# lashhw/rtcuda

Measured on AMD Instinct MI355X. Metric: Msamples/s at 1920x1080, bun_zipper.ply, higher is better.
Workload: dtype f32

## Files before the change

### rtcuda_amd/api.py

```python
from __future__ import annotations

import ctypes
import dataclasses
import os
import subprocess

import numpy as np

from .scenes import SceneArrays

_PKG = os.path.dirname(os.path.abspath(__file__))
LIB_PATH = os.path.join(_PKG, os.environ.get("RT_LIB_NAME", "librtcuda_amd.so"))
CSRC = os.path.join(_PKG, "csrc")

W = 1 << 20
FLAG_TIME_KERNELS = 1
FLAG_DETERMINISTIC = 2
FLAG_RNG_PER_SAMPLE = 4
FLAG_REFERENCE_WALK = 8
SCENE_DEVICE_BVH = 1
FLAG_WATERTIGHT = 16
AOV_CHANNELS = 11
AOV_ALBEDO, AOV_NORMAL, AOV_EMISSION, AOV_DEPTH, AOV_HITS = 0, 3, 6, 9, 10

# ... 20 lines not shown


class RtStats(ctypes.Structure):
    _fields_ = [
        ("camera_rays", ctypes.c_int64), ("shade_events", ctypes.c_int64), ("closest_rays", ctypes.c_int64),
        ("any_rays", ctypes.c_int64), ("emission_adds", ctypes.c_int64), ("shadow_adds", ctypes.c_int64),
        ("rr_draws", ctypes.c_int64), ("iterations", ctypes.c_int64), ("bvh_nodes", ctypes.c_int64),
        ("bvh_depth", ctypes.c_int64), ("seconds_render", ctypes.c_double), ("seconds_rng_init", ctypes.c_double),
        ("seconds_trace", ctypes.c_double), ("seconds_reference_tree", ctypes.c_double), ("seconds_advance", ctypes.c_double),
        ("launches_trace", ctypes.c_int64), ("reserved", ctypes.c_int64 * 7),
    ]

    def as_dict(self) -> dict:
        d = {n: getattr(self, n) for n, _ in self._fields_ if n != "reserved"}
        d["lds_top_records"] = int(self.reserved[2])
        d["slot_chunk"] = max(int(self.reserved[1]) - 1, 0)
        d["literal_retraces"], d["reference_lost_hits"], d["exact_ties"] = (int(self.reserved[k]) for k in (4, 5, 6))
        return d


class RtDenoiseParams(ctypes.Structure):
    _fields_ = [("passes", ctypes.c_int32), ("sigma_color", ctypes.c_float), ("sigma_depth", ctypes.c_float),
                ("normal_power_log2", ctypes.c_int32), ("flags", ctypes.c_uint32)]


class RtDenoiseDualParams(ctypes.Structure):
    _fields_ = [("passes", ctypes.c_int32), ("sigma_variance", ctypes.c_float), ("sigma_depth", ctypes.c_float),
                ("normal_power_log2", ctypes.c_int32), ("flags", ctypes.c_uint32)]


def build(verbose: bool = False) -> str:
# ... 813 lines not shown
```

### rtcuda_amd/csrc/rt_frame_kernels.inc

```

template <bool LDS_TABLES>
__global__ void __launch_bounds__(kBlock)
RT_K_ADVANCE(DScene sc, DPools p, RT_FRAME_SRC cam, AdvanceParams ap, float *__restrict__ fb, DCounters *__restrict__ ctr,
             DWaveRow *__restrict__ rows, unsigned int *__restrict__ lock_shades) {
    if (ap.lockstep >= 3 && lock_shades[ap.lockstep - 2] == 0u) return;
    __shared__ float s_tab[LDS_TABLES ? kTabDwordsMax : 1];
    const int i = blockIdx.x * blockDim.x + threadIdx.x;
    const bool in_range = i < ap.n;
    SlotState st;
    st.bounces = kDone;
    st.hit_info = -1;
    st.pixel = 0;
    st.gen = 0;
    st.rs = Rng{0, 0, 0, 0, 0, 0};
    st.beta = st.wo = st.isect_p = st.isect_n = mk(0, 0, 0);
    if (in_range) {
        st.bounces = p.bounces(i);
        st.hit_info = p.hit_info(i);
        st.pixel = p.pixel(i);
        st.gen = p.gen(i);
        st.rs = Rng{p.rd(i), p.r0(i), p.r1(i), p.r2(i), p.r3(i), p.r4(i)};
        st.beta = mk(p.br(i), p.bg(i), p.bb(i));
        st.wo = mk(p.dx(i), p.dy(i), p.dz(i));
        st.isect_p = mk(p.hpx(i), p.hpy(i), p.hpz(i));
// ... 84 lines not shown
           int prio_period, int rot_wave, int rot_set, int gen_batch, int tri_follow, unsigned int *__restrict__ next_cid,
           unsigned long long *__restrict__ vstat) {
    constexpr bool SPLIT_GEN = MIN_WAVES != 2;
    asm volatile("s_nop 0\n\ts_nop 0");
    extern __shared__ int s_lds[];
    int *stack = s_lds + threadIdx.x;
    float *park = (float *)(s_lds + (stack_cap + 1) * kBlock) + threadIdx.x;
    int *over = overflow + (blockIdx.x * kBlock + threadIdx.x) % kOverStride;
    int *cold = s_lds + (stack_cap + 10) * kBlock + threadIdx.x;
    float *acc = (float *)(s_lds + (stack_cap + 23) * kBlock) + threadIdx.x;
    float *s_tab = (float *)(s_lds + (stack_cap + 26) * kBlock);
    const float *tab = sc.tables;
    const float4 *s_top = (const float4 *)(s_tab + (LDS_TABLES ? ((sc.tab_dwords + 3) & ~3) : 0));
    constexpr bool CHUNKS = RT_PATHS_CHUNKS && SPLIT_GEN && !DRAW_CIDS;
    __shared__ __attribute__((aligned(16))) unsigned s_task[CHUNKS ? 8 : 1];
    if (CHUNKS && threadIdx.x == 0) {
        const rtchunks::Multiple m = rtchunks::multiple_of(top_n > 0 ? (unsigned)top_n : 1u);
        s_task[0] = 0u;
        s_task[1] = top_n > 0 ? (unsigned)top_n : 0u;
        s_task[2] = m.inv;
        s_task[3] = m.shift;
        s_task[4] = m.limit;
    }
    const bool chunk_start = CHUNKS && top_n > 0;
    if (MIN_WAVES != 2) top_n = 0;
    for (int k = threadIdx.x; k < top_n * 4; k += kBlock) ((float4 *)s_top)[k] = sc.nodes[k];
    if (LDS_TABLES) {
        for (int k = threadIdx.x; k < sc.tab_dwords; k += kBlock) s_tab[k] = sc.tables[k];
        tab = s_tab;
    }
    struct Uniforms {
        RT_FRAME_SRC cam;
        AdvanceParams ap;
    };
    static_assert(sizeof(Uniforms) % 4 == 0, "dword copy");
    Uniforms *s_uni = (Uniforms *)(s_top + 4 * (size_t)top_n);
    {
        Uniforms u;
        u.cam = cam_arg;
// ... 88 lines not shown
    acc[0 * kBlock] = acc[1 * kBlock] = acc[2 * kBlock] = 0.f;
    if (chunk_start) {
        i = ap_n;
        phase = PH_GEN;
        cold[12 * kBlock] = -1;
    } else if (i < ap_n) {
        load_slot(i);
        phase = (bounces != kDone && bounces != kParked) ? (SPLIT_GEN ? PH_GEN : PH_ADV) : PH_IDLE;
        cold_save();
        cold[12 * kBlock] = -1;
    }
    unsigned long long n_gen = 0, n_shade = 0, n_traced = 0, n_shadow = 0, n_emit = 0, n_deposit = 0, n_rr = 0;
#ifdef RT_TRACE_PROFILE
    unsigned long long pf[16] = {0, 0, 0, 0, 0, 0, 0, 0, 0, 0, 0, 0, 0, 0, 0, 0};
    unsigned long long pf_gen_cycles = 0, pf_fin_cycles = 0, pf_fin_lanes = 0, pf_fin_iters = 0;
    const unsigned long long pf_t0 = __builtin_readcyclecounter();
    unsigned long long pf_last_work = 0;
#endif

    unsigned prio_tick = 0;
    const unsigned prio_rank = (4u * blockIdx.x) / gridDim.x;
    while (true) {
        RT_MARK("loop.head");
        if (prio_period && (prio_tick++ & ((1u << prio_period) - 1u)) == 0u) {
            unsigned lvl = ((prio_tick >> prio_period) + prio_rank) & 3u;
            lvl = max(lvl, prio_rank >> 1);
            switch (lvl) {
                case 0: __builtin_amdgcn_s_setprio(0); break;
                case 1: __builtin_amdgcn_s_setprio(1); break;
                case 2: __builtin_amdgcn_s_setprio(2); break;
// ... 36 lines not shown
                while (served < need) {
                    if (cid_next == cid_end) {
                        unsigned base = 0;
                        if (lane_id() == 0) base = atomicAdd(next_cid, (unsigned)kCidChunk);
                        static_assert(0x7ffff000u + (unsigned)kCidChunk < 0x7fffffffu, "cid_end must not overflow int");
                        cid_next = (int)min(__builtin_amdgcn_readfirstlane(base), 0x7ffff000u);
                        cid_end = cid_next + kCidChunk;
                    }
                    const int take = min(need - served, cid_end - cid_next);
                    if (phase == PH_GEN && rank >= served && rank < served + take) my_cid = cid_next + (rank - served);
                    cid_next += take;
                    served += take;
                }
            }
            const unsigned chunk_g = CHUNKS ? __builtin_amdgcn_readfirstlane(s_task[1]) : 0u;
            if (CHUNKS && chunk_g) {
                const rtchunks::Multiple chunk_m{s_task[2], s_task[3], s_task[4]};
                bool need = phase == PH_GEN && i >= ap_n;
                const bool at_end = phase == PH_GEN && i < ap_n &&
                                    rtchunks::chunk_ends((unsigned)cold[2 * kBlock], chunk_m, cold[0 * kBlock] == kChunkFresh);
                if (wave_ballot(need || at_end)) {
                    if (at_end) {
                        cold_load();
                        const bool ends = gen == ap.last_gen || (long long)gen * kW + (ap.slot_lo + i) >= ap.cam_end;
                        if (!ends) {
                            acc_flush(acc, fb, ap_fb_fixed, pixel);
                            bounces = ap_max_bounces;
                            store_slot(i);
                            const int old = __hip_atomic_fetch_add(&p.sem(i), 1, __ATOMIC_RELEASE, __HIP_MEMORY_SCOPE_WORKGROUP);
                            if (!rtchunks::runner_keeps(old)) {
                                i = ap_n;
                                need = true;
                            }
                        }
                    }
                    const unsigned chunk_sets = (unsigned)ap_n / (unsigned)lanes_in_grid;
                    const unsigned chunk_tasks = rtchunks::task_count(chunk_sets, (unsigned)ap.last_gen, (unsigned)chunk_g);
                    unsigned long long m;
                    while ((m = wave_ballot(need)) != 0ull) {
                        unsigned base = 0;
                        if (lane_id() == 0) base = atomicAdd(&s_task[0], (unsigned)__popcll(m));
                        const unsigned t = __builtin_amdgcn_readfirstlane(base) + prefix_popc(m);
                        if (need) {
                            if (t >= chunk_tasks) {
                                need = false;
                                phase = PH_IDLE;
                            } else {
                                const rtchunks::Entry e = rtchunks::task_entry(t, chunk_sets);
                                const int k = slot_of((int)e.set, e.lane);
                                const int old = k < ap_n ? __hip_atomic_fetch_sub(&p.sem(k), 1, __ATOMIC_ACQUIRE, __HIP_MEMORY_SCOPE_WORKGROUP) : 0;
                                if (rtchunks::taker_runs(old)) {
                                    i = k;
                                    load_slot(i);
                                    cold_save();
                                    cold[0 * kBlock] = kChunkFresh;
                                    cold[12 * kBlock] = -1;
                                    need = false;
                                }
                            }
                        }
                    }
                }
            }
            if (phase == PH_GEN) {
                SlotState st;
                st.gen = cold[2 * kBlock];
                st.rs = Rng{(uint32_t)cold[3 * kBlock], (uint32_t)cold[4 * kBlock], (uint32_t)cold[5 * kBlock],
                            (uint32_t)cold[6 * kBlock], (uint32_t)cold[7 * kBlock], (uint32_t)cold[8 * kBlock]};
                st.bounces = 0;
                st.pixel = 0;
                st.beta = mk(0, 0, 0);
                int pxy = cold[12 * kBlock];
                acc_flush(acc, fb, ap_fb_fixed, cold[1 * kBlock]);
                gen_core<true>(cam, ap, ap.slot_lo + i, st, out, &pxy, my_cid);
                cold[0 * kBlock] = st.bounces;
                cold[2 * kBlock] = st.gen;
                cold[3 * kBlock] = (int)st.rs.d;
                cold[4 * kBlock] = (int)st.rs.v0;
                cold[5 * kBlock] = (int)st.rs.v1;
                cold[6 * kBlock] = (int)st.rs.v2;
                cold[7 * kBlock] = (int)st.rs.v3;
                cold[8 * kBlock] = (int)st.rs.v4;
                if (out.new_ray) {
                    cold[1 * kBlock] = st.pixel;
                    cold[9 * kBlock] = __float_as_int(st.beta.x);
                    cold[10 * kBlock] = __float_as_int(st.beta.y);
                    cold[11 * kBlock] = __float_as_int(st.beta.z);
                    cold[12 * kBlock] = pxy;
// ... 2 lines not shown
                }
            }
            const bool nr = out.new_ray;
            o = out.ray_o;
            d = out.ray_d;
            inv = inv_dir(d);
            phase = nr ? (int)PH_CLOSEST : phase;
            tmax = nr ? kFltMax : tmax;
            tri = nr ? -1 : tri;
            cur = nr ? 0 : cur;
            sp = nr ? 0 : sp;
            if (wave_ballot(hand_back)) {
                if (hand_back) {
                    if (draw_cids) {
                        phase = PH_IDLE;
                    } else if (CHUNKS && chunk_g) {
                        cold_load();
                        store_slot(i);
                        i = ap_n;
                        tri = -1;
                    } else {
                        next_slot(PH_GEN);
                    }
                }
            }
            n_gen += wave_count((out.did_gen));
            n_traced += wave_count((out.new_ray));
#ifdef RT_TRACE_PROFILE
            pf_gen_cycles += __builtin_readcyclecounter() - pf_tg;
#endif
            retake();
            RT_MARK("gen.end");
        }
        if (run_adv) {
#ifdef RT_TRACE_PROFILE
// ... 275 lines not shown
        pf_last_work = phase != PH_IDLE ? pf_tf - pf_t0 : pf_last_work;
#endif
    }
#ifdef RT_TRACE_PROFILE
    if (prof && lane_id() == 0) { atomicAdd(&prof[17], pf_fin_cycles); atomicAdd(&prof[18], pf_fin_lanes); atomicAdd(&prof[19], pf_fin_iters); }
    const unsigned long long pf_life = __builtin_readcyclecounter() - pf_t0;
    unsigned long long pf_idle = pf_life - pf_last_work, pf_idle_max = pf_idle;
    for (int off = 32; off > 0; off >>= 1) {
        pf_idle += __shfl_xor(pf_idle, off);
        const unsigned long long other = __shfl_xor(pf_idle_max, off);
        pf_idle_max = other > pf_idle_max ? other : pf_idle_max;
    }
    if (prof && lane_id() == 0)
        { pf[11] = pf_life; for (int k = 0; k < 16; k++) atomicAdd(&prof[k], pf[k]); atomicMax(&prof[13], pf[11]); atomicAdd(&prof[14], 1ull); atomicAdd(&prof[16], pf_gen_cycles);
          atomicAdd(&prof[20], pf_idle); atomicAdd(&prof[21], pf_idle_max);
          unsigned long long *rec = prof + 24 + kProfRec * (size_t)((blockIdx.x * kBlock + threadIdx.x) >> 6);
          rec[0] = __builtin_amdgcn_s_getreg((31 << 11) | 4);
          rec[1] = __builtin_amdgcn_s_getreg((31 << 11) | 20);
          rec[2] = pf[11];
          rec[3] = pf[0] + pf[2] + pf[4];
          rec[4] = pf_idle;
          rec[5] = pf_idle_max; }
#endif
    unsigned long long v[C_COUNT] = {n_gen, n_shade, n_traced, n_shadow, n_emit, n_deposit, n_rr, 0ull};
    row_add(rows, v);
}
```

### rtcuda_amd/csrc/rt_host_check.cpp

```cpp
#include <cfloat>
#include <cmath>
#include <cstdint>
#include <cstdio>
#include <cstring>
#include <cstdlib>
#include <vector>

#include "rt_bvh.h"
#include "rt_denoise.h"
#include "rt_launch_plan.h"
#include "rt_ploc.h"
#include "rt_ref_tree.h"
#include "rt_slot_chunks.h"
#include "rt_stats_merge.h"

namespace {
struct V3 { float x, y, z; };
inline V3 sub(V3 a, V3 b) { return {a.x - b.x, a.y - b.y, a.z - b.z}; }
inline float dot(V3 a, V3 b) { return a.x * b.x + a.y * b.y + a.z * b.z; }
inline V3 cross(V3 a, V3 b) { return {a.y * b.z - a.z * b.y, a.z * b.x - a.x * b.z, a.x * b.y - a.y * b.x}; }
struct Tri { V3 p0, e1, e2, n; };
inline bool tri_hit(const Tri &tr, V3 o, V3 d, float tmax, float &t) {
    V3 c = sub(tr.p0, o);
    V3 r = cross(d, c);
// ... 837 lines not shown
        slots[k] = rtchunks::slot_of(e.set, (unsigned)block * rtchunks::kLanes + e.lane, (unsigned)lanes_in_grid, (unsigned)rot_wave, (unsigned)rot_set);
        levels[k] = (int32_t)e.level;
    }
}
int rt_slot_chunk_static_slot(int set, int lane_in_grid, int lanes_in_grid, int rot_wave, int rot_set) {
    return rtchunks::slot_of((unsigned)set, (unsigned)lane_in_grid, (unsigned)lanes_in_grid, (unsigned)rot_wave, (unsigned)rot_set);
}
uint32_t rt_slot_chunk_levels(uint32_t rays, uint32_t G) { return rtchunks::levels(rays, G); }
uint32_t rt_slot_chunk_task_count(uint32_t sets, uint32_t rays, uint32_t G) { return rtchunks::task_count(sets, rays, G); }
int rt_slot_chunk_ends(uint32_t gen, uint32_t G, int fresh) { return rtchunks::chunk_ends(gen, rtchunks::multiple_of(G), fresh != 0); }
int rt_slot_chunk_taker_runs(int old_sem) { return rtchunks::taker_runs(old_sem); }
int rt_slot_chunk_runner_keeps(int old_sem) { return rtchunks::runner_keeps(old_sem); }
int rt_plan_slot_chunk(int n, int cus, int chain) {
    return rtplan::slot_chunk_for(rtplan::plan_paths_launch(n, cus, true, 70000, 10, true, 1920, 256, 0), chain);
}
int hc_denoise(const int64_t *sum_fixed, int num_samples, const int64_t *aov_fixed, int aov_samples, int width, int height, int passes,
               float sigma_color, float sigma_depth, int normal_power_log2, float *rgb_out) {
    if (!sum_fixed || !aov_fixed || !rgb_out || width < 1 || height < 1 || num_samples < 1 || aov_samples < 1) return 1;
    if (passes < 0 || passes > DN_MAX_PASSES || normal_power_log2 < 0 || normal_power_log2 > DN_MAX_NORMAL_POWER_LOG2) return 1;
    if (!(std::isfinite(sigma_color) && sigma_color > 0.f && std::isfinite(sigma_depth) && sigma_depth > 0.f)) return 1;
    const float sc2 = sigma_color * sigma_color, sd2 = sigma_depth * sigma_depth;
    const float kz = 1.f / sd2;
    float kc[DN_MAX_PASSES];
    for (int i = 0; i < passes; i++) {
        kc[i] = (float)(1 << (2 * i)) / sc2;
        if (!(std::isfinite(kc[i]) && kc[i] > 0.f)) return 1;
    }
    if (!(std::isfinite(kz) && kz > 0.f)) return 1;
    const size_t n = (size_t)width * (size_t)height;
    const float inv_spp = 1.f / (float)num_samples, inv_aov = 1.f / (float)aov_samples;
// ... 44 lines not shown
```

### rtcuda_amd/csrc/rt_host_render.inc

```
struct Context {
    int device = -1;
    int n = 0;
    int lane = 0;
    DPools pools{};
    std::vector<void *> allocs;
    DCounters *d_ctr = nullptr;
    DCounters *h_ctr = nullptr;
    DWaveRow *d_rows = nullptr;
    int n_rows = 0;
    uint32_t *d_jump = nullptr;
    hipEvent_t ev_ring[4] = {nullptr, nullptr, nullptr, nullptr};
    hipEvent_t ev_a = nullptr, ev_b = nullptr, ev_c = nullptr;
    uint64_t rng_seed = 0;
    int rng_lo = -1;
    bool rng_valid = false;
    uint32_t *rng_backup = nullptr;
    std::vector<hipEvent_t> timing_events;
    unsigned int *d_lock = nullptr;
    int lock_cap = 0;
    int *d_over = nullptr;
    int over_levels = 0;
    std::mutex busy;
    Context() = default;
    Context(const Context &) = delete;
// ... 206 lines not shown
    RayTable table;
    long long n_rays;
    bool keyed = false;
    KeyedRayTable keyed_table{};
};
struct FrameRun {
    Context &c;
    const rt_scene *scene;
    const RayFrame *rays;
    hipStream_t st;
    float *d_sum;
    uint32_t flags;
    bool per_sample;
    HitMode mode;
    bool lds_tables = false, persistent = true, finished = false, ran_lockstep = false;
    int cus = 0, stack_cap = 0, top_records_in_lds = 0, slot_chunk = 0, lock_enqueued = 0;
    DScene sc{};
    Camera cam{};
    AdvanceParams ap{};
    TraceParams tpp{};
    size_t lds_bytes = 0, ev_used = 0;
    dim3 grid_trace;
    TraceKernel trace = nullptr;
    hipEvent_t ev_start = nullptr, ev_stop = nullptr;
    long long rounds = 0;
    float ms_paths = 0.f;
    double rng_seconds = 0.0, ref_tree_seconds = 0.0;
    ~FrameRun() {
        if (ev_start) (void)hipEventDestroy(ev_start);
        if (ev_stop) (void)hipEventDestroy(ev_stop);
    }
// ... 12 lines not shown
        }
        *out = c.timing_events[ev_used++];
        return 0;
    }
};

#ifdef RT_TRACE_PROFILE
static int report_paths_profile(unsigned long long *paths_prof, int paths_blocks) {
    unsigned long long h[24];
    HIP_TRY(hipMemcpy(h, paths_prof, 192, hipMemcpyDeviceToHost));
    fprintf(stderr, "k_paths cycles: ADV %.1f%% (%.0f / block) node %.1f%% (%.0f) tri %.1f%% (%.0f) rest %.1f%%\n",
            100.0 * h[8] / h[11], h[0] ? (double)h[8] / h[0] : 0.0, 100.0 * h[9] / h[11], h[2] ? (double)h[9] / h[2] : 0.0,
            100.0 * h[10] / h[11], h[4] ? (double)h[10] / h[4] : 0.0, 100.0 * (double)(h[11] - h[8] - h[9] - h[10]) / h[11]);
    fprintf(stderr, "k_paths GEN blocks: %llu avg lanes %.1f, %.1f %% of wave time (%.0f cycles / block; inside `rest` above)\n", h[12],
            h[12] ? (double)h[15] / h[12] : 0.0, 100.0 * h[16] / h[11], h[12] ? (double)h[16] / h[12] : 0.0);
    fprintf(stderr, "k_paths waves: %llu, mean lifetime %.0f cycles, longest %.0f cycles (x%.3f)\n", h[14], (double)h[11] / h[14], (double)h[13],
            (double)h[13] * h[14] / h[11]);
    fprintf(stderr, "k_paths lane-idle tail: %.2f %% of wave time x 64 lanes; a wave's first lane is idle for good %.2f %% of the wave's time before its exit\n",
            100.0 * h[20] / (64.0 * h[11]), 100.0 * h[21] / h[11]);
    fprintf(stderr, "k_paths fin section: %.1f %% of wave time, entered in %llu iterations (avg %.1f finished lanes), %.0f cycles each\n",
            100.0 * h[17] / h[11], h[19], h[19] ? (double)h[18] / h[19] : 0.0, h[19] ? (double)h[17] / h[19] : 0.0);
    fprintf(stderr, "k_paths profile: ADV blocks %llu avg lanes %.1f | node steps %llu avg lanes %.1f (ADV-waiting %.1f) | tri steps %llu avg lanes %.1f (ADV-waiting %.1f)\n",
            h[0], h[0] ? (double)h[1] / h[0] : 0.0, h[2], h[2] ? (double)h[3] / h[2] : 0.0, h[2] ? (double)h[6] / h[2] : 0.0, h[4],
            h[4] ? (double)h[5] / h[4] : 0.0, h[4] ? (double)h[7] / h[4] : 0.0);
    if (const char *dump = knob("RT_PROF_DUMP")) {
        std::vector<unsigned long long> recs(kProfRec * (size_t)paths_blocks * (kBlock / 64));
        HIP_TRY(hipMemcpy(recs.data(), paths_prof + 24, recs.size() * 8, hipMemcpyDeviceToHost));
        if (FILE *f = fopen(dump, "w")) {
            for (size_t k = 0; k < recs.size(); k += kProfRec)
                fprintf(f, "%zu %llu %llu %llu %llu %llu %llu\n", k / kProfRec, recs[k], recs[k + 1], recs[k + 2], recs[k + 3], recs[k + 4], recs[k + 5]);
// ... 20 lines not shown
    const size_t fixed_lds = (lds_tables ? sizeof(float) * (size_t)((scene->tab_dwords + 3) & ~3) : 0) + sizeof(Camera) + sizeof(AdvanceParams);
    const rtplan::PathsLaunch p = rtplan::plan_paths_launch(c.n, cus, scene->wide, scene->n_nodes, paths_cap, !rays, ap.width, ap.spp, fixed_lds);
    top_records_in_lds = p.top_n;
    unsigned long long *paths_prof = nullptr;
#ifdef RT_TRACE_PROFILE
    const size_t prof_bytes = 192 + 8 * kProfRec * (size_t)(grid_for(c.n) * (kBlock / 64));
    HIP_TRY(hipMalloc((void **)&paths_prof, prof_bytes));
    HIP_TRY(hipMemset(paths_prof, 0, prof_bytes));
#endif
    auto launch_paths = [&](auto kernel, const auto &src, int top_n) {
        hipLaunchKernelGGL(kernel, dim3(p.blocks), dim3(kBlock), p.lds_bytes, st, sc, c.pools, src, ap, d_sum, c.d_rows, paths_cap, c.d_over,
                           p.adv_batch, (flags & 0x100u) ? 1 : 0, paths_prof, top_n, p.prio_rotate, p.rot_wave, p.rot_set, p.gen_batch, p.tri_follow, &c.d_ctr->pad2[0],
                           &c.d_ctr->vstat[0]);
    };
    HIP_TRY(hipEventRecord(c.ev_a, st));
    const int chunk = (rays || p.few_blocks || per_sample || ap.last_gen < 1 || ap.n != c.n) ? 0 : rtplan::slot_chunk_for(p, ap.last_gen);
    slot_chunk = chunk;
    if (rays && rays->keyed) launch_paths(paths_keyed_kernel(lds_tables, p.few_blocks), rays->keyed_table, p.top_n);
    else if (rays) launch_paths(paths_rays_kernel(lds_tables, p.few_blocks, mode.verify), rays->table, p.top_n);
    else if (chunk > 0) launch_paths(paths_chunked_kernel(lds_tables, scene->wide, mode.literal, mode.verify), cam, chunk);
    else launch_paths(paths_kernel(lds_tables, scene->wide, p.few_blocks, per_sample, mode.literal, mode.verify), cam, mode.literal ? 0 : p.top_n);
    HIP_TRY(hipGetLastError());
    HIP_TRY(hipEventRecord(c.ev_b, st));
    HIP_TRY(hipEventSynchronize(c.ev_b));
    HIP_TRY(hipEventElapsedTime(&ms_paths, c.ev_a, c.ev_b));
#ifdef RT_TRACE_PROFILE
    if (report_paths_profile(paths_prof, p.blocks)) return 1;
#endif
    finished = true;
    return 0;
}

int FrameRun::run_rounds() {
    const int kBatch = 8;
    const int kTimeStride = 4;
// ... 112 lines not shown
    stats->bvh_nodes = scene->n_nodes;
    stats->bvh_depth = scene->max_depth;
    stats->seconds_render = ms_total * 1e-3;
    stats->seconds_rng_init = rng_seconds;
    double scale_up = n_sampled > 0 ? (double)rounds / (double)n_sampled : 0.0;
    stats->seconds_trace = t_ch * 1e-3 * scale_up;
    stats->seconds_reference_tree = ref_tree_seconds;
    stats->seconds_advance = t_adv * 1e-3 * scale_up;
    stats->launches_trace = rounds;
    stats->reserved[0] = n_sampled;
    if (persistent) {
        stats->seconds_trace = ms_paths * 1e-3;
        stats->seconds_advance = 0.0;
        stats->launches_trace = 1;
        stats->reserved[0] = 1;
        stats->reserved[1] = 1 + slot_chunk;
        stats->reserved[2] = top_records_in_lds;
    }
    rare_path_counters(h_final.vstat, &stats->reserved[4]);
    return 0;
}

int render_shard_impl(const rt_scene *scene, const rt_camera *camera, int width, int height, int spp,
                      int max_bounces, uint64_t seed, int shard_index, int shard_count, uint32_t flags,
                      float *d_sum, hipStream_t st, rt_stats *stats, int ctx_lane = 0, const RayFrame *rays = nullptr) {
    if (!scene || (!camera && !rays) || !d_sum) return fail("rt_render_shard: null argument");
    if (width <= 0 || height <= 0 || spp <= 0 || max_bounces < 0) return fail("rt_render_shard: bad dimensions");
    if (max_bounces > (1 << 24)) return fail("rt_render_shard: max_bounces exceeds 16777216");
    if (shard_count <= 0 || kW % shard_count != 0 || shard_index < 0 || shard_index >= shard_count)
        return fail("rt_render_shard: shard_count must divide 1048576 and 0 <= shard_index < shard_count");
    if ((long long)width * height > (long long)(0x7fffffff / 3))
// ... 389 lines not shown
```

### rtcuda_amd/csrc/rt_launch_plan.h

```cpp
#pragma once

#include <algorithm>
#include <cstdlib>

#include "rt_bvh.h"

namespace rtplan {
constexpr int kBlock = 256, kSlots = 1 << 20;

struct PathsLaunch {
    int blocks;
    bool few_blocks;
    size_t lds_bytes;
    int top_n, adv_batch, gen_batch, tri_follow, prio_rotate, rot_wave, rot_set;
    int slot_chunk;
};
constexpr int kSlotChunkAuto = -1, kChunksPerSlot = 8, kChunkChainLo = 384, kChunkChainHi = 768;

inline PathsLaunch plan_paths_launch(int n, int cus, bool wide, int n_nodes, int paths_cap, bool lattice, int width, int spp,
                                     size_t fixed_lds_bytes) {
    using rtbvh::knob;
    PathsLaunch p{};
    p.lds_bytes = sizeof(int) * (size_t)kBlock * (size_t)(paths_cap + 26) + fixed_lds_bytes;
    p.blocks = (n + kBlock - 1) / kBlock;
    {
        int want = 1024;
        if (const char *e = knob("RT_PATHS_BLOCKS")) want = std::max(1, atoi(e));
        while (p.blocks > want && p.blocks % 2 == 0) p.blocks /= 2;
    }
    p.few_blocks = p.blocks <= 2 * cus;
    if (p.few_blocks) {
        const int prefix = std::min(n_nodes, (int)rtbvh::kTopPrefix * (wide ? 2 : 1));
// ... 19 lines not shown
            while (b) { long long t = a % b; a = b; b = t; }
            period = a * (spp / 64);
        }
        const int waves = p.blocks * (kBlock / 64);
        if (period < 16 || period > waves) period = std::max(16, waves / 8);
        p.rot_wave = (int)(period / 4);
        p.rot_set = (int)(period / 4 + period / 16);
        if (const char *e = knob("RT_ROT_WAVE")) p.rot_wave = atoi(e);
        if (const char *e = knob("RT_ROT_SET")) p.rot_set = atoi(e);
        p.rot_wave &= ~3;
    }
    if (const char *e = knob("RT_PRIO_ROTATE")) p.prio_rotate = atoi(e);
    p.slot_chunk = (p.few_blocks || n / (p.blocks * kBlock) < 2) ? 0 : kSlotChunkAuto;
    if (const char *e = knob("RT_SLOT_CHUNK")) p.slot_chunk = p.few_blocks ? 0 : std::max(0, std::min(1 << 20, atoi(e)));
    if (n % (p.blocks * kBlock) != 0) p.slot_chunk = 0;
    return p;
}
inline int slot_chunk_for(const PathsLaunch &p, int chain) {
    if (p.slot_chunk != kSlotChunkAuto) return p.slot_chunk;
    if (chain < kChunkChainLo || chain > kChunkChainHi) return 0;
    return (chain + kChunksPerSlot - 1) / kChunksPerSlot;
}
}
```

### rtcuda_amd/csrc/rt_slot_chunks.h

```cpp
#pragma once

#if defined(__HIPCC__)
#define RT_CHUNKS_FN __host__ __device__ inline
#else
#define RT_CHUNKS_FN inline
#endif

namespace rtchunks {
constexpr unsigned kLanes = 256;

RT_CHUNKS_FN unsigned levels(unsigned rays, unsigned G) { return (rays + G - 1u) / G; }
RT_CHUNKS_FN unsigned task_count(unsigned sets, unsigned rays, unsigned G) { return sets * kLanes * levels(rays, G); }

struct Entry {
    unsigned set, lane, level;
};
RT_CHUNKS_FN Entry task_entry(unsigned t, unsigned sets) {
    const unsigned S = sets * kLanes, idx = t % S;
    return Entry{idx / kLanes, idx % kLanes, t / S};
}

RT_CHUNKS_FN int slot_of(unsigned set, unsigned lane_in_grid, unsigned lanes_in_grid, unsigned rot_wave, unsigned rot_set) {
    const unsigned wave_in_grid = lane_in_grid >> 6, lane_in_wave = lane_in_grid & 63u;
    const unsigned b = (wave_in_grid + (wave_in_grid & 3u) * rot_wave + set * rot_set) & ((lanes_in_grid >> 6) - 1u);
    return (int)(set * lanes_in_grid + b * 64u + lane_in_wave);
}

RT_CHUNKS_FN bool taker_runs(int old_sem) { return old_sem >= 1; }
RT_CHUNKS_FN bool runner_keeps(int old_sem) { return old_sem < 0; }

struct Multiple {
    unsigned inv, shift, limit;
};
RT_CHUNKS_FN Multiple multiple_of(unsigned G) {
    unsigned shift = 0;
    while (((G >> shift) & 1u) == 0u) shift++;
    const unsigned odd = G >> shift;
    unsigned inv = odd;
    for (int k = 0; k < 5; k++) inv *= 2u - odd * inv;
    return Multiple{inv, shift, 0xffffffffu / G};
}
RT_CHUNKS_FN bool is_multiple(unsigned gen, const Multiple &m) {
    const unsigned q = gen * m.inv;
    return ((q >> m.shift) | (m.shift ? q << (32u - m.shift) : 0u)) <= m.limit;
}
// ... 3 lines not shown
```

### rtcuda_amd/csrc/rtcuda_amd.hip

```cpp
#include <hip/hip_runtime.h>

#include <algorithm>
#include <chrono>
#include <cmath>
#include <cstdio>
#include <cstring>
#include <memory>
#include <mutex>
#include <thread>
#include <type_traits>
#include <string>
#include <vector>

#include "../../include/rtcuda_amd.h"
#include "rt_bvh.h"
#include "rt_denoise.h"
#include "rt_device.h"
#include "rt_launch_plan.h"
#include "rt_ploc.h"
#include "rt_ref_tree.h"
#include "rt_slot_chunks.h"
#include "rt_stats_merge.h"

using namespace rt;
// ... 39 lines not shown
    const float *tables;
    int tab_dwords;
    const float4 *ref_nodes;
    const int *ref_prims;
    int ref_n_prims;
    const int *ref_leaf_of;
    const int *ref_parent;
    int ref_root_leaf;
};
__device__ __host__ inline int tab_off_lights(int n_mats) { return 5 * n_mats; }
__device__ __host__ inline int tab_off_ltri(int n_mats, int n_lights) { return 5 * n_mats + 8 * n_lights; }
__device__ __host__ inline int tab_off_lpre(int n_mats, int n_lights) { return 5 * n_mats + 20 * n_lights; }
constexpr int kTabPerMat = 5, kTabPerLight = 8 + 12 + 4;
inline int tab_dwords(int n_mats, int n_lights) { return kTabPerMat * n_mats + kTabPerLight * n_lights; }

enum { A_OX, A_OY, A_OZ, A_DX, A_DY, A_DZ, A_HPX, A_HPY, A_HPZ, A_HNX, A_HNY, A_HNZ, A_BR, A_BG, A_BB, A_SOX, A_SOY, A_SOZ, A_SDX, A_SDY, A_SDZ, A_STMAX, A_SLR, A_SLG, A_SLB, A_HIT_INFO, A_BOUNCES, A_PIXEL, A_GEN, A_STARGET, A_RD, A_R0, A_R1, A_R2, A_R3, A_R4, A_SEM, A_COUNT };
struct DPools {
    float *base;
    int n;
    __device__ __forceinline__ float &ox(int i) const { return base[(unsigned)(A_OX * n + i)]; }
    __device__ __forceinline__ float &oy(int i) const { return base[(unsigned)(A_OY * n + i)]; }
    __device__ __forceinline__ float &oz(int i) const { return base[(unsigned)(A_OZ * n + i)]; }
    __device__ __forceinline__ float &dx(int i) const { return base[(unsigned)(A_DX * n + i)]; }
    __device__ __forceinline__ float &dy(int i) const { return base[(unsigned)(A_DY * n + i)]; }
    __device__ __forceinline__ float &dz(int i) const { return base[(unsigned)(A_DZ * n + i)]; }
    __device__ __forceinline__ float &hpx(int i) const { return base[(unsigned)(A_HPX * n + i)]; }
    __device__ __forceinline__ float &hpy(int i) const { return base[(unsigned)(A_HPY * n + i)]; }
    __device__ __forceinline__ float &hpz(int i) const { return base[(unsigned)(A_HPZ * n + i)]; }
    __device__ __forceinline__ float &hnx(int i) const { return base[(unsigned)(A_HNX * n + i)]; }
    __device__ __forceinline__ float &hny(int i) const { return base[(unsigned)(A_HNY * n + i)]; }
    __device__ __forceinline__ float &hnz(int i) const { return base[(unsigned)(A_HNZ * n + i)]; }
// ... 9 lines not shown
    __device__ __forceinline__ float &stmax(int i) const { return base[(unsigned)(A_STMAX * n + i)]; }
    __device__ __forceinline__ float &slr(int i) const { return base[(unsigned)(A_SLR * n + i)]; }
    __device__ __forceinline__ float &slg(int i) const { return base[(unsigned)(A_SLG * n + i)]; }
    __device__ __forceinline__ float &slb(int i) const { return base[(unsigned)(A_SLB * n + i)]; }
    __device__ __forceinline__ int &hit_info(int i) const { return ((int *)base)[(unsigned)(A_HIT_INFO * n + i)]; }
    __device__ __forceinline__ int &bounces(int i) const { return ((int *)base)[(unsigned)(A_BOUNCES * n + i)]; }
    __device__ __forceinline__ int &pixel(int i) const { return ((int *)base)[(unsigned)(A_PIXEL * n + i)]; }
    __device__ __forceinline__ int &gen(int i) const { return ((int *)base)[(unsigned)(A_GEN * n + i)]; }
    __device__ __forceinline__ int &starget(int i) const { return ((int *)base)[(unsigned)(A_STARGET * n + i)]; }
    __device__ __forceinline__ uint32_t &rd(int i) const { return ((uint32_t *)base)[(unsigned)(A_RD * n + i)]; }
    __device__ __forceinline__ uint32_t &r0(int i) const { return ((uint32_t *)base)[(unsigned)(A_R0 * n + i)]; }
    __device__ __forceinline__ uint32_t &r1(int i) const { return ((uint32_t *)base)[(unsigned)(A_R1 * n + i)]; }
    __device__ __forceinline__ uint32_t &r2(int i) const { return ((uint32_t *)base)[(unsigned)(A_R2 * n + i)]; }
    __device__ __forceinline__ uint32_t &r3(int i) const { return ((uint32_t *)base)[(unsigned)(A_R3 * n + i)]; }
    __device__ __forceinline__ uint32_t &r4(int i) const { return ((uint32_t *)base)[(unsigned)(A_R4 * n + i)]; }
    __device__ __forceinline__ int &sem(int i) const { return ((int *)base)[(unsigned)(A_SEM * n + i)]; }
    float *array(int k) const { return base + (size_t)k * n; }
};

struct DCounters {
    int last_live_round;
    unsigned int unused0;
    unsigned int pad2[2];
    unsigned long long vstat[4];
};
enum { V_OWN_FAIL = 0, V_LOST = 1, V_TIE = 2, V_LITERAL = 3 };
enum { C_CAMERA = 0, C_SHADE, C_CLOSEST, C_ANY, C_EMIT, C_SHADOW_ADD, C_RR, C_UNUSED, C_COUNT };
struct DWaveRow {
    unsigned long long c[C_COUNT];
};

// ... 46 lines not shown
    p.rd(i) = seed_state.d;
    p.r0(i) = v[0];
    p.r1(i) = v[1];
    p.r2(i) = v[2];
    p.r3(i) = v[3];
    p.r4(i) = v[4];
}

__global__ void k_pool_init(DPools p, int n, int max_bounces) {
    int i = blockIdx.x * blockDim.x + threadIdx.x;
    if (i >= n) return;
    p.hit_info(i) = -1;
    p.bounces(i) = max_bounces;
    p.gen(i) = 0;
    p.pixel(i) = 0;
    p.sem(i) = 1;
}

struct AdvanceParams {
    int n;
    int slot_lo;
    int width, height, spp, max_bounces;
    long long cam_end;
    int round;
    int batch_mask;
    int last_gen;
    int lockstep;
    int fb_fixed;
    int w_over_spp;
    int dpx, dpy;
    int per_sample, key_mul, key_add;
// ... 770 lines not shown
```

Baseline: 5053.

## Move chunk hand-off semaphores into LDS and deal only the tail slot sets

Replaces the per-slot global semaphore array with packed 16-bit LDS semaphore fields, so release and acquire become workgroup-local LDS atomics instead of global memory atomics. Chunked dealing now applies only to the last few slot sets (a 'head' offset packed into top_n), and the accumulator flush is deferred until after the hand-off. Chunking is disabled unless occupancy allows enough resident workgroups per CU. The catch is that hand-offs are restricted to within a workgroup and to fewer sets, and there is an extra waitcnt before the release atomic.

Result: faster. 5110, median of 6 (+1.1%).

```diff
diff --git a/rtcuda_amd/api.py b/rtcuda_amd/api.py
--- a/rtcuda_amd/api.py
+++ b/rtcuda_amd/api.py
@@ -58,7 +58,8 @@
     def as_dict(self) -> dict:
         d = {n: getattr(self, n) for n, _ in self._fields_ if n != "reserved"}
         d["lds_top_records"] = int(self.reserved[2])
-        d["slot_chunk"] = max(int(self.reserved[1]) - 1, 0)
+        d["slot_chunk"] = max((int(self.reserved[1]) & 0xffffffff) - 1, 0)
+        d["slot_head"] = int(self.reserved[1]) >> 32
         d["literal_retraces"], d["reference_lost_hits"], d["exact_ties"] = (int(self.reserved[k]) for k in (4, 5, 6))
         return d
 
diff --git a/rtcuda_amd/csrc/rt_frame_kernels.inc b/rtcuda_amd/csrc/rt_frame_kernels.inc
--- a/rtcuda_amd/csrc/rt_frame_kernels.inc
+++ b/rtcuda_amd/csrc/rt_frame_kernels.inc
@@ -1,3 +1,6 @@
+#ifndef RT_CHUNK_RELEASE_WAIT
+#define RT_CHUNK_RELEASE_WAIT 1
+#endif
 
 template <bool LDS_TABLES>
 __global__ void __launch_bounds__(kBlock)
@@ -122,15 +125,22 @@
     const float4 *s_top = (const float4 *)(s_tab + (LDS_TABLES ? ((sc.tab_dwords + 3) & ~3) : 0));
     constexpr bool CHUNKS = RT_PATHS_CHUNKS && SPLIT_GEN && !DRAW_CIDS;
     __shared__ __attribute__((aligned(16))) unsigned s_task[CHUNKS ? 8 : 1];
-    if (CHUNKS && threadIdx.x == 0) {
-        const rtchunks::Multiple m = rtchunks::multiple_of(top_n > 0 ? (unsigned)top_n : 1u);
-        s_task[0] = 0u;
-        s_task[1] = top_n > 0 ? (unsigned)top_n : 0u;
-        s_task[2] = m.inv;
-        s_task[3] = m.shift;
-        s_task[4] = m.limit;
-    }
-    const bool chunk_start = CHUNKS && top_n > 0;
+    __shared__ unsigned s_sem[CHUNKS ? rtchunks::kSemWords : 1];
+    const unsigned chunk_g0 = (CHUNKS && top_n > 0) ? (unsigned)top_n & ((1u << rtplan::kChunkHeadShift) - 1u) : 0u;
+    const unsigned chunk_head0 = (CHUNKS && top_n > 0) ? (unsigned)top_n >> rtplan::kChunkHeadShift : 0u;
+    if (CHUNKS) {
+        for (unsigned k = threadIdx.x; k < rtchunks::kSemWords; k += kBlock) s_sem[k] = rtchunks::kSemWordInit;
+        if (threadIdx.x == 0) {
+            const rtchunks::Multiple m = rtchunks::multiple_of(chunk_g0 ? chunk_g0 : 1u);
+            s_task[0] = 0u;
+            s_task[1] = chunk_g0;
+            s_task[2] = m.inv;
+            s_task[3] = m.shift;
+            s_task[4] = m.limit;
+            s_task[5] = chunk_head0;
+        }
+    }
+    const bool chunk_start = CHUNKS && chunk_g0 && chunk_head0 == 0u;
     if (MIN_WAVES != 2) top_n = 0;
     for (int k = threadIdx.x; k < top_n * 4; k += kBlock) ((float4 *)s_top)[k] = sc.nodes[k];
     if (LDS_TABLES) {
@@ -249,6 +259,7 @@
 #ifdef RT_TRACE_PROFILE
     unsigned long long pf[16] = {0, 0, 0, 0, 0, 0, 0, 0, 0, 0, 0, 0, 0, 0, 0, 0};
     unsigned long long pf_gen_cycles = 0, pf_fin_cycles = 0, pf_fin_lanes = 0, pf_fin_iters = 0;
+    unsigned long long pf_handovers = 0, pf_handover_blocks = 0;
     const unsigned long long pf_t0 = __builtin_readcyclecounter();
     unsigned long long pf_last_work = 0;
 #endif
@@ -315,27 +326,45 @@
                 }
             }
             const unsigned chunk_g = CHUNKS ? __builtin_amdgcn_readfirstlane(s_task[1]) : 0u;
+            const bool chunk_was_gen = CHUNKS && phase == PH_GEN;
+            const int chunk_acc_pixel = CHUNKS ? cold[1 * kBlock] : 0;
             if (CHUNKS && chunk_g) {
                 const rtchunks::Multiple chunk_m{s_task[2], s_task[3], s_task[4]};
+                const unsigned chunk_head = __builtin_amdgcn_readfirstlane(s_task[5]);
                 bool need = phase == PH_GEN && i >= ap_n;
-                const bool at_end = phase == PH_GEN && i < ap_n &&
+                const bool at_end = phase == PH_GEN && i < ap_n && slot_set >= (int)chunk_head &&
                                     rtchunks::chunk_ends((unsigned)cold[2 * kBlock], chunk_m, cold[0 * kBlock] == kChunkFresh);
                 if (wave_ballot(need || at_end)) {
+#ifdef RT_TRACE_PROFILE
+                    bool pf_released = false;
+#endif
                     if (at_end) {
                         cold_load();
                         const bool ends = gen == ap.last_gen || (long long)gen * kW + (ap.slot_lo + i) >= ap.cam_end;
                         if (!ends) {
-                            acc_flush(acc, fb, ap_fb_fixed, pixel);
                             bounces = ap_max_bounces;
                             store_slot(i);
-                            const int old = __hip_atomic_fetch_add(&p.sem(i), 1, __ATOMIC_RELEASE, __HIP_MEMORY_SCOPE_WORKGROUP);
-                            if (!rtchunks::runner_keeps(old)) {
+                            const rtchunks::Owner own = rtchunks::owner_of((unsigned)i, (unsigned)lanes_in_grid, (unsigned)rot_wave, (unsigned)rot_set);
+                            const unsigned idx = (own.set - chunk_head) * rtchunks::kLanes + (own.lane_in_grid & (rtchunks::kLanes - 1u));
+#if RT_CHUNK_RELEASE_WAIT
+                            __builtin_amdgcn_s_waitcnt(0x0f70);
+#endif
+                            const unsigned old = __hip_atomic_fetch_add(&s_sem[rtchunks::sem_word(idx) & (rtchunks::kSemWords - 1u)], rtchunks::sem_unit(idx),
+                                                                        __ATOMIC_RELEASE, __HIP_MEMORY_SCOPE_WORKGROUP);
+                            if (!rtchunks::runner_keeps(rtchunks::sem_value(old, idx))) {
                                 i = ap_n;
                                 need = true;
                             }
+#ifdef RT_TRACE_PROFILE
+                            pf_released = true;
+#endif
                         }
                     }
-                    const unsigned chunk_sets = (unsigned)ap_n / (unsigned)lanes_in_grid;
+#ifdef RT_TRACE_PROFILE
+                    pf_handovers += wave_count(pf_released);
+                    pf_handover_blocks += wave_ballot(pf_released) != 0 ? 1 : 0;
+#endif
+                    const unsigned chunk_sets = (unsigned)ap_n / (unsigned)lanes_in_grid - chunk_head;
                     const unsigned chunk_tasks = rtchunks::task_count(chunk_sets, (unsigned)ap.last_gen, (unsigned)chunk_g);
                     unsigned long long m;
                     while ((m = wave_ballot(need)) != 0ull) {
@@ -348,9 +377,12 @@
                                 phase = PH_IDLE;
                             } else {
                                 const rtchunks::Entry e = rtchunks::task_entry(t, chunk_sets);
-                                const int k = slot_of((int)e.set, e.lane);
-                                const int old = k < ap_n ? __hip_atomic_fetch_sub(&p.sem(k), 1, __ATOMIC_ACQUIRE, __HIP_MEMORY_SCOPE_WORKGROUP) : 0;
-                                if (rtchunks::taker_runs(old)) {
+                                const int k = slot_of((int)(e.set + chunk_head), e.lane);
+                                const unsigned idx = e.set * rtchunks::kLanes + e.lane;
+                                const unsigned old = k < ap_n ? __hip_atomic_fetch_sub(&s_sem[rtchunks::sem_word(idx) & (rtchunks::kSemWords - 1u)], rtchunks::sem_unit(idx),
+                                                                                       __ATOMIC_ACQUIRE, __HIP_MEMORY_SCOPE_WORKGROUP)
+                                                              : rtchunks::kSemBias;
+                                if (rtchunks::taker_runs(rtchunks::sem_value(old, idx))) {
                                     i = k;
                                     load_slot(i);
                                     cold_save();
@@ -363,6 +395,10 @@
                     }
                 }
             }
+            if (CHUNKS) {
+                __builtin_amdgcn_s_waitcnt(0x0f70);
+                if (chunk_was_gen) acc_flush(acc, fb, ap_fb_fixed, chunk_acc_pixel);
+            }
             if (phase == PH_GEN) {
                 SlotState st;
                 st.gen = cold[2 * kBlock];
@@ -372,7 +408,7 @@
                 st.pixel = 0;
                 st.beta = mk(0, 0, 0);
                 int pxy = cold[12 * kBlock];
-                acc_flush(acc, fb, ap_fb_fixed, cold[1 * kBlock]);
+                if (!CHUNKS) acc_flush(acc, fb, ap_fb_fixed, cold[1 * kBlock]);
                 gen_core<true>(cam, ap, ap.slot_lo + i, st, out, &pxy, my_cid);
                 cold[0 * kBlock] = st.bounces;
                 cold[2 * kBlock] = st.gen;
@@ -405,11 +441,12 @@
                 if (hand_back) {
                     if (draw_cids) {
                         phase = PH_IDLE;
-                    } else if (CHUNKS && chunk_g) {
+                    } else if (CHUNKS && chunk_g && slot_set + 1 >= (int)s_task[5]) {
                         cold_load();
                         store_slot(i);
                         i = ap_n;
                         tri = -1;
+                        slot_set = (int)s_task[5];
                     } else {
                         next_slot(PH_GEN);
                     }
@@ -715,6 +752,7 @@
     if (prof && lane_id() == 0)
         { pf[11] = pf_life; for (int k = 0; k < 16; k++) atomicAdd(&prof[k], pf[k]); atomicMax(&prof[13], pf[11]); atomicAdd(&prof[14], 1ull); atomicAdd(&prof[16], pf_gen_cycles);
           atomicAdd(&prof[20], pf_idle); atomicAdd(&prof[21], pf_idle_max);
+          atomicAdd(&prof[22], pf_handovers); atomicAdd(&prof[23], pf_handover_blocks);
           unsigned long long *rec = prof + 24 + kProfRec * (size_t)((blockIdx.x * kBlock + threadIdx.x) >> 6);
           rec[0] = __builtin_amdgcn_s_getreg((31 << 11) | 4);
           rec[1] = __builtin_amdgcn_s_getreg((31 << 11) | 20);
diff --git a/rtcuda_amd/csrc/rt_host_check.cpp b/rtcuda_amd/csrc/rt_host_check.cpp
--- a/rtcuda_amd/csrc/rt_host_check.cpp
+++ b/rtcuda_amd/csrc/rt_host_check.cpp
@@ -875,6 +875,30 @@
 int rt_plan_slot_chunk(int n, int cus, int chain) {
     return rtplan::slot_chunk_for(rtplan::plan_paths_launch(n, cus, true, 70000, 10, true, 1920, 256, 0), chain);
 }
+int rt_plan_slot_head(int n, int cus, int *sets_out) {
+    const rtplan::PathsLaunch p = rtplan::plan_paths_launch(n, cus, true, 70000, 10, true, 1920, 256, 0);
+    const int sets = n / (p.blocks * rtplan::kBlock);
+    if (sets_out) *sets_out = sets;
+    return rtplan::slot_head_for(p, sets);
+}
+int rt_plan_slot_chunk_if_resident(int chunk, int workgroups_per_cu) { return rtplan::slot_chunk_if_resident(chunk, workgroups_per_cu); }
+void rt_slot_chunk_head_tasks(int block, int sets, int head, int lanes_in_grid, int rot_wave, int rot_set, uint32_t t0, int count, int32_t *slots, int32_t *levels, int32_t *idx) {
+    for (int k = 0; k < count; k++) {
+        const rtchunks::Entry e = rtchunks::task_entry(t0 + (uint32_t)k, (unsigned)(sets - head));
+        slots[k] = rtchunks::slot_of(e.set + (unsigned)head, (unsigned)block * rtchunks::kLanes + e.lane, (unsigned)lanes_in_grid, (unsigned)rot_wave, (unsigned)rot_set);
+        levels[k] = (int32_t)e.level;
+        idx[k] = (int32_t)(e.set * rtchunks::kLanes + e.lane);
+    }
+}
+void rt_slot_chunk_owner(int slot, int lanes_in_grid, int rot_wave, int rot_set, int32_t *out2) {
+    const rtchunks::Owner o = rtchunks::owner_of((unsigned)slot, (unsigned)lanes_in_grid, (unsigned)rot_wave, (unsigned)rot_set);
+    out2[0] = (int32_t)o.set;
+    out2[1] = (int32_t)o.lane_in_grid;
+}
+uint32_t rt_slot_chunk_sem_word(uint32_t idx) { return rtchunks::sem_word(idx); }
+uint32_t rt_slot_chunk_sem_unit(uint32_t idx) { return rtchunks::sem_unit(idx); }
+int rt_slot_chunk_sem_value(uint32_t word, uint32_t idx) { return rtchunks::sem_value(word, idx); }
+uint32_t rt_slot_chunk_sem_init() { return rtchunks::kSemWordInit; }
 int hc_denoise(const int64_t *sum_fixed, int num_samples, const int64_t *aov_fixed, int aov_samples, int width, int height, int passes,
                float sigma_color, float sigma_depth, int normal_power_log2, float *rgb_out) {
     if (!sum_fixed || !aov_fixed || !rgb_out || width < 1 || height < 1 || num_samples < 1 || aov_samples < 1) return 1;
diff --git a/rtcuda_amd/csrc/rt_host_render.inc b/rtcuda_amd/csrc/rt_host_render.inc
--- a/rtcuda_amd/csrc/rt_host_render.inc
+++ b/rtcuda_amd/csrc/rt_host_render.inc
@@ -244,7 +244,7 @@
     bool per_sample;
     HitMode mode;
     bool lds_tables = false, persistent = true, finished = false, ran_lockstep = false;
-    int cus = 0, stack_cap = 0, top_records_in_lds = 0, slot_chunk = 0, lock_enqueued = 0;
+    int cus = 0, stack_cap = 0, top_records_in_lds = 0, slot_chunk = 0, slot_head = 0, lock_enqueued = 0;
     DScene sc{};
     Camera cam{};
     AdvanceParams ap{};
@@ -287,6 +287,8 @@
             100.0 * h[10] / h[11], h[4] ? (double)h[10] / h[4] : 0.0, 100.0 * (double)(h[11] - h[8] - h[9] - h[10]) / h[11]);
     fprintf(stderr, "k_paths GEN blocks: %llu avg lanes %.1f, %.1f %% of wave time (%.0f cycles / block; inside `rest` above)\n", h[12],
             h[12] ? (double)h[15] / h[12] : 0.0, 100.0 * h[16] / h[11], h[12] ? (double)h[16] / h[12] : 0.0);
+    fprintf(stderr, "k_paths GEN cycles per wave %.0f; chunked deal: %.2f hand-overs per lane, made in %.2f %% of the GEN blocks\n", h[14] ? (double)h[16] / h[14] : 0.0,
+            h[14] ? (double)h[22] / (64.0 * h[14]) : 0.0, h[12] ? 100.0 * h[23] / h[12] : 0.0);
     fprintf(stderr, "k_paths waves: %llu, mean lifetime %.0f cycles, longest %.0f cycles (x%.3f)\n", h[14], (double)h[11] / h[14], (double)h[13],
             (double)h[13] * h[14] / h[11]);
     fprintf(stderr, "k_paths lane-idle tail: %.2f %% of wave time x 64 lanes; a wave's first lane is idle for good %.2f %% of the wave's time before its exit\n",
@@ -337,11 +339,19 @@
                            &c.d_ctr->vstat[0]);
     };
     HIP_TRY(hipEventRecord(c.ev_a, st));
-    const int chunk = (rays || p.few_blocks || per_sample || ap.last_gen < 1 || ap.n != c.n) ? 0 : rtplan::slot_chunk_for(p, ap.last_gen);
+    int chunk = (rays || p.few_blocks || per_sample || ap.last_gen < 1 || ap.n != c.n) ? 0 : rtplan::slot_chunk_for(p, ap.last_gen);
+    const PathsKernel chunked = paths_chunked_kernel(lds_tables, scene->wide, mode.literal, mode.verify);
+    if (chunk > 0) {
+        int per_cu = 0;
+        HIP_TRY(hipOccupancyMaxActiveBlocksPerMultiprocessor(&per_cu, chunked, kBlock, p.lds_bytes));
+        chunk = rtplan::slot_chunk_if_resident(chunk, per_cu);
+    }
+    slot_head = chunk > 0 ? rtplan::slot_head_for(p, ap.n / (p.blocks * kBlock)) : 0;
+    static_assert(rtplan::kDealtSetsMax == (int)rtchunks::kDealtSetsMax, "the plan deals what the semaphores hold");
     slot_chunk = chunk;
     if (rays && rays->keyed) launch_paths(paths_keyed_kernel(lds_tables, p.few_blocks), rays->keyed_table, p.top_n);
     else if (rays) launch_paths(paths_rays_kernel(lds_tables, p.few_blocks, mode.verify), rays->table, p.top_n);
-    else if (chunk > 0) launch_paths(paths_chunked_kernel(lds_tables, scene->wide, mode.literal, mode.verify), cam, chunk);
+    else if (chunk > 0) launch_paths(chunked, cam, chunk | (slot_head << rtplan::kChunkHeadShift));
     else launch_paths(paths_kernel(lds_tables, scene->wide, p.few_blocks, per_sample, mode.literal, mode.verify), cam, mode.literal ? 0 : p.top_n);
     HIP_TRY(hipGetLastError());
     HIP_TRY(hipEventRecord(c.ev_b, st));
@@ -484,7 +494,7 @@
         stats->seconds_advance = 0.0;
         stats->launches_trace = 1;
         stats->reserved[0] = 1;
-        stats->reserved[1] = 1 + slot_chunk;
+        stats->reserved[1] = 1 + slot_chunk + ((int64_t)slot_head << 32);
         stats->reserved[2] = top_records_in_lds;
     }
     rare_path_counters(h_final.vstat, &stats->reserved[4]);
diff --git a/rtcuda_amd/csrc/rt_launch_plan.h b/rtcuda_amd/csrc/rt_launch_plan.h
--- a/rtcuda_amd/csrc/rt_launch_plan.h
+++ b/rtcuda_amd/csrc/rt_launch_plan.h
@@ -14,8 +14,11 @@
     size_t lds_bytes;
     int top_n, adv_batch, gen_batch, tri_follow, prio_rotate, rot_wave, rot_set;
     int slot_chunk;
+    int slot_head;
 };
 constexpr int kSlotChunkAuto = -1, kChunksPerSlot = 8, kChunkChainLo = 384, kChunkChainHi = 768;
+constexpr int kSlotHeadAuto = -1, kDealtSetsDefault = 2, kDealtSetsMax = 4, kChunkWorkgroupsPerCu = 4;
+constexpr int kChunkHeadShift = 21, kChunkSetsMax = 1 << (31 - kChunkHeadShift);
 
 inline PathsLaunch plan_paths_launch(int n, int cus, bool wide, int n_nodes, int paths_cap, bool lattice, int width, int spp,
                                      size_t fixed_lds_bytes) {
@@ -65,8 +68,16 @@
     p.slot_chunk = (p.few_blocks || n / (p.blocks * kBlock) < 2) ? 0 : kSlotChunkAuto;
     if (const char *e = knob("RT_SLOT_CHUNK")) p.slot_chunk = p.few_blocks ? 0 : std::max(0, std::min(1 << 20, atoi(e)));
     if (n % (p.blocks * kBlock) != 0) p.slot_chunk = 0;
+    if (n / (p.blocks * kBlock) > kChunkSetsMax) p.slot_chunk = 0;
+    p.slot_head = kSlotHeadAuto;
+    if (const char *e = knob("RT_SLOT_HEAD")) p.slot_head = std::max(0, atoi(e));
     return p;
 }
+inline int slot_head_for(const PathsLaunch &p, int sets) {
+    const int head = p.slot_head == kSlotHeadAuto ? sets - kDealtSetsDefault : p.slot_head;
+    return std::max(std::max(0, sets - kDealtSetsMax), std::min(head, sets - 1));
+}
+inline int slot_chunk_if_resident(int chunk, int workgroups_per_cu) { return workgroups_per_cu >= kChunkWorkgroupsPerCu ? chunk : 0; }
 inline int slot_chunk_for(const PathsLaunch &p, int chain) {
     if (p.slot_chunk != kSlotChunkAuto) return p.slot_chunk;
     if (chain < kChunkChainLo || chain > kChunkChainHi) return 0;
diff --git a/rtcuda_amd/csrc/rt_slot_chunks.h b/rtcuda_amd/csrc/rt_slot_chunks.h
--- a/rtcuda_amd/csrc/rt_slot_chunks.h
+++ b/rtcuda_amd/csrc/rt_slot_chunks.h
@@ -29,6 +29,26 @@
 RT_CHUNKS_FN bool taker_runs(int old_sem) { return old_sem >= 1; }
 RT_CHUNKS_FN bool runner_keeps(int old_sem) { return old_sem < 0; }
 
+constexpr unsigned kSemBias = 0x4000u, kSemBanked = kSemBias + 1u;
+constexpr unsigned kSemWordInit = kSemBanked | (kSemBanked << 16);
+constexpr unsigned kDealtSetsMax = 4;
+constexpr unsigned kSemWords = kDealtSetsMax * kLanes / 2u;
+static_assert(kSemBias > 2046u && kSemBias + 1u < 0x10000u, "a field must hold [bias - 2046, bias + 1]");
+RT_CHUNKS_FN unsigned sem_word(unsigned idx) { return idx >> 1; }
+RT_CHUNKS_FN unsigned sem_unit(unsigned idx) { return 1u << (16u * (idx & 1u)); }
+RT_CHUNKS_FN int sem_value(unsigned word, unsigned idx) { return (int)((word >> (16u * (idx & 1u))) & 0xffffu) - (int)kSemBias; }
+
+struct Owner {
+    unsigned set, lane_in_grid;
+};
+RT_CHUNKS_FN Owner owner_of(unsigned slot, unsigned lanes_in_grid, unsigned rot_wave, unsigned rot_set) {
+    const unsigned mask = (lanes_in_grid >> 6) - 1u;
+    const unsigned set = slot >> (31u - (unsigned)__builtin_clz(lanes_in_grid)), b = (slot >> 6) & mask;
+    const unsigned low = (b - set * rot_set) & 3u;
+    const unsigned wave = (b - low * rot_wave - set * rot_set) & mask;
+    return Owner{set, wave * 64u + (slot & 63u)};
+}
+
 struct Multiple {
     unsigned inv, shift, limit;
 };
diff --git a/rtcuda_amd/csrc/rtcuda_amd.hip b/rtcuda_amd/csrc/rtcuda_amd.hip
--- a/rtcuda_amd/csrc/rtcuda_amd.hip
+++ b/rtcuda_amd/csrc/rtcuda_amd.hip
@@ -77,7 +77,7 @@
 constexpr int kTabPerMat = 5, kTabPerLight = 8 + 12 + 4;
 inline int tab_dwords(int n_mats, int n_lights) { return kTabPerMat * n_mats + kTabPerLight * n_lights; }
 
-enum { A_OX, A_OY, A_OZ, A_DX, A_DY, A_DZ, A_HPX, A_HPY, A_HPZ, A_HNX, A_HNY, A_HNZ, A_BR, A_BG, A_BB, A_SOX, A_SOY, A_SOZ, A_SDX, A_SDY, A_SDZ, A_STMAX, A_SLR, A_SLG, A_SLB, A_HIT_INFO, A_BOUNCES, A_PIXEL, A_GEN, A_STARGET, A_RD, A_R0, A_R1, A_R2, A_R3, A_R4, A_SEM, A_COUNT };
+enum { A_OX, A_OY, A_OZ, A_DX, A_DY, A_DZ, A_HPX, A_HPY, A_HPZ, A_HNX, A_HNY, A_HNZ, A_BR, A_BG, A_BB, A_SOX, A_SOY, A_SOZ, A_SDX, A_SDY, A_SDZ, A_STMAX, A_SLR, A_SLG, A_SLB, A_HIT_INFO, A_BOUNCES, A_PIXEL, A_GEN, A_STARGET, A_RD, A_R0, A_R1, A_R2, A_R3, A_R4, A_COUNT };
 struct DPools {
     float *base;
     int n;
@@ -117,7 +117,6 @@
     __device__ __forceinline__ uint32_t &r2(int i) const { return ((uint32_t *)base)[(unsigned)(A_R2 * n + i)]; }
     __device__ __forceinline__ uint32_t &r3(int i) const { return ((uint32_t *)base)[(unsigned)(A_R3 * n + i)]; }
     __device__ __forceinline__ uint32_t &r4(int i) const { return ((uint32_t *)base)[(unsigned)(A_R4 * n + i)]; }
-    __device__ __forceinline__ int &sem(int i) const { return ((int *)base)[(unsigned)(A_SEM * n + i)]; }
     float *array(int k) const { return base + (size_t)k * n; }
 };
 
@@ -194,7 +193,6 @@
     p.bounces(i) = max_bounces;
     p.gen(i) = 0;
     p.pixel(i) = 0;
-    p.sem(i) = 1;
 }
 
 struct AdvanceParams {
```
